# soedinglab/spacedust

Measured on AMD Instinct MI355X. Metric: clustersearch throughput (genome-pairs/s; SW GCUPS alongside), higher is better.
Workload: dtype int16

## Files before the change

include/spacedust_gpu.h:

```cpp
#ifndef SPACEDUST_GPU_H
#define SPACEDUST_GPU_H

#include <stddef.h>
#include <stdint.h>

#ifdef __cplusplus
extern "C" {
#endif

enum {
    SD_OK = 0,
    SD_ENODEVICE = -1,
    SD_EHIP = -2,
    SD_EINVAL = -3,
    SD_ENOMEM = -4,
    SD_EUNSUPPORTED = -5,
    SD_EMISMATCH = -6
};

typedef struct sd_ctx sd_ctx;
typedef struct sd_seqset sd_seqset;
typedef struct sd_target sd_target;

int sd_ctx_create(int device, sd_ctx **out);
// ... 48 lines not shown
                              uint32_t nPairs, const uint32_t *pairQ, const uint32_t *pairT, const uint8_t *isIdentity,
                              uint32_t *outIdx, sd_sw_result *out, uint32_t *nOut, char *btPool, uint64_t btCap,
                              uint64_t *btUsed);

int sd_sw_align_batch_compact_diag(sd_ctx *ctx, const sd_sw_params *par, const sd_seqset *queries, const sd_seqset *targets,
                                   uint32_t nPairs, const uint32_t *pairQ, const uint32_t *pairT, const uint16_t *pairDiag,
                                   const uint8_t *isIdentity, uint32_t *outIdx, sd_sw_result *out, uint32_t *nOut, char *btPool,
                                   uint64_t btCap, uint64_t *btUsed);

int sd_seqset_set_groups(sd_seqset *s, const uint32_t *groupOf, uint32_t nGroups, const uint32_t *keys);
int sd_sw_align_batch_best_by_group(sd_ctx *ctx, const sd_sw_params *par, const sd_seqset *queries, const sd_seqset *targets,
                                    uint32_t nPairs, const uint32_t *pairQ, const uint32_t *pairT, const uint16_t *pairDiag,
                                    const uint8_t *isIdentity, float seqIdThr, int32_t alnLenThr, uint32_t *outIdx, sd_sw_result *out,
                                    uint32_t *nOut, char *btPool, uint64_t btCap, uint64_t *btUsed);

int sd_sw_align_alt_batch(sd_ctx *ctx, const sd_sw_params *par, const sd_seqset *queries, const sd_seqset *targets, uint32_t nSeeds,
                          const uint32_t *seedQ, const uint32_t *seedT, const int32_t *tStart, const int32_t *tEnd,
                          const uint8_t *isIdentity, uint32_t maxAlt, float seqIdThr, int32_t alnLenThr, int32_t seqIdMode,
                          sd_sw_result *out, uint32_t *outCount, char *btPool, uint64_t btCap, uint64_t *btUsed);
int sd_sw_alt_last_stats(sd_ctx *ctx, uint64_t *groups, uint64_t *seedRounds, uint64_t *bytesCopied);

int sd_sw_set_cigar_pool(sd_ctx *ctx, int on);
int sd_sw_download_bytes(sd_ctx *ctx, uint64_t *recordBytes, uint64_t *poolBytes);

int sd_selftest_sort_pairs(sd_ctx *ctx, const uint32_t *keys, const uint32_t *vals, uint32_t n, int beginBit, int endBit, uint32_t *outKeys,
                           uint32_t *outVals);
int sd_selftest_scan(sd_ctx *ctx, const uint32_t *in, uint32_t n, uint64_t *exclusiveSum, uint32_t *runningMax);
int sd_selftest_r2p_weights(sd_ctx *ctx, uint32_t nTasks, const uint32_t *nRows, const uint32_t *L, const uint8_t *cells, float *freq,
                            float *eff);

int sd_sw_align_batch_hostpath(sd_ctx *ctx, const sd_sw_params *par, const sd_seqset *queries, const sd_seqset *targets,
                               uint32_t nPairs, const uint32_t *pairQ, const uint32_t *pairT, const uint8_t *isIdentity,
                               sd_sw_result *out, char *btPool, uint64_t btCap, uint64_t *btUsed);

int sd_sw_score_batch(sd_ctx *ctx, const sd_sw_params *par, const sd_seqset *queries, const sd_seqset *targets,
                      uint32_t nPairs, const uint32_t *pairQ, const uint32_t *pairT, int lanes, int reverse,
                      const int32_t *qEnd, const int32_t *tEnd, int32_t *out);

int sd_sw_last_cells(sd_ctx *ctx, uint64_t *forwardCells, uint64_t *reverseCells, uint64_t *tracebackCells);

typedef struct {
    int32_t kmerSize;
    int32_t kmerThr;
    int32_t maxHitsPerQuery;
    int32_t minDiagScore;
    uint32_t binSize;
// ... 343 lines not shown
```

spacedust_amd/_lib.py:

```python
import ctypes as C
import os

import numpy as np

HERE = os.path.dirname(os.path.abspath(__file__))
LIB_PATH = os.path.join(HERE, 'libsdgpu.so')

_vp = C.c_void_p


SD_OK, SD_ENODEVICE, SD_EHIP, SD_EINVAL, SD_ENOMEM, SD_EUNSUPPORTED, SD_EMISMATCH = 0, -1, -2, -3, -4, -5, -6


class SdError(RuntimeError):
    pass


class SwParams(C.Structure):
    _fields_ = [('gapOpen', C.c_int32), ('gapExtend', C.c_int32), ('matrix', C.c_int8 * 441), ('covMode', C.c_int32),
                ('covThr', C.c_float), ('evalThr', C.c_double), ('swMode', C.c_int32), ('dbResidues', C.c_uint64)]


class SwResult(C.Structure):
    _fields_ = [('score', C.c_int32), ('qStart', C.c_int32), ('qEnd', C.c_int32), ('tStart', C.c_int32),
# ... 196 lines not shown
        'sd_search_create_indexed': (C.c_int, [C.c_int, C.POINTER(SearchParams), C.POINTER(SetDbView), C.POINTER(IndexView), C.POINTER(_vp)]),
        'sd_search_destroy': (None, [_vp]),
        'sd_search_last_error': (C.c_char_p, [_vp]),
        'sd_search_ctx': (_vp, [_vp, C.c_int]),
        'sd_search_target': (_vp, [_vp]),
        'sd_search_set_sinks': (C.c_int, [_vp, _vp, _vp, _vp]),
        'sd_search_set_chunk_queries': (C.c_int, [_vp, C.c_int32]),
        'sd_search_set_want_records': (C.c_int, [_vp, C.c_int]),
        'sd_search_stream': (C.c_int, [_vp, C.POINTER(SetDbView), C.c_int, C.c_uint32, _vp, _vp, _vp]),
        'sd_search_result_counts': (C.c_int, [_vp, _vp]),
        'sd_search_result_arrays': (C.c_int, [_vp] + [_vp] * 12),
        'sd_search_result_write_tsv': (C.c_int, [_vp, C.c_char_p, C.c_char_p, _vp, C.c_char_p, _vp, C.c_char_p, _vp, C.c_char_p, _vp,
                                                 C.c_int, C.c_int, C.c_uint64, C.POINTER(C.c_uint64), C.POINTER(C.c_uint64)]),
        'sd_search_result_records': (C.c_int, [_vp, _vp, C.c_uint64, C.POINTER(C.c_uint64)]),
        'sd_agg_records': (C.c_int, [_vp] * 7 + [_vp, C.c_uint64, C.POINTER(C.c_uint64)]),
        'sd_records_check': (C.c_int, [_vp, C.c_uint64, C.c_uint32, C.c_uint32, C.c_uint32, C.c_uint32, C.POINTER(C.c_uint64), C.POINTER(C.c_uint64)]),
        'sd_records_write_tsv': (C.c_int, [_vp, C.c_uint64, C.c_char_p, C.c_int, C.c_uint64, C.c_char_p, _vp, C.c_char_p, _vp, C.c_char_p, _vp,
                                           C.c_char_p, _vp, C.c_int, C.POINTER(C.c_uint64), C.POINTER(C.c_uint64)]),
        'sd_search_result_destroy': (None, [_vp]),
        'sd_search_stats': (C.c_int, [_vp, _vp, _vp]),
        'sd_search_download_bytes': (C.c_int, [_vp, C.POINTER(C.c_uint64), C.POINTER(C.c_uint64)]),
        'sd_sw_set_cigar_pool': (C.c_int, [_vp, C.c_int]),
        'sd_sw_download_bytes': (C.c_int, [_vp, C.POINTER(C.c_uint64), C.POINTER(C.c_uint64)]),
        'sd_r2p_create': (C.c_int, [C.POINTER(_vp)]),
        'sd_r2p_destroy': (None, [_vp]),
        'sd_r2p_batch': (C.c_int, [_vp, C.POINTER(R2pParams), C.c_uint32] + [_vp] * 12),
        'sd_r2p_batch_device': (C.c_int, [_vp, _vp, C.POINTER(R2pParams), C.c_uint32] + [_vp] * 12),
        'sd_selftest_r2p_weights': (C.c_int, [_vp, C.c_uint32, _vp, _vp, _vp, _vp, _vp]),
        'sd_shard_query_sets': (C.c_int, [_vp, C.c_uint32, C.c_uint32, C.c_uint32, _vp, C.POINTER(C.c_uint32)]),
        'sd_comm_unique_id': (C.c_int, [C.c_char_p]),
        'sd_comm_init': (C.c_int, [C.c_int, C.c_int, C.c_int, C.c_char_p, C.POINTER(_vp)]),
        'sd_comm_destroy': (None, [_vp]),
        'sd_comm_host_buffer': (C.c_int, [_vp, C.c_int, C.c_uint64, C.POINTER(_vp)]),
        'sd_comm_last_error': (C.c_char_p, [_vp]),
        'sd_search_set_records_sink': (C.c_int, [_vp, _vp, _vp]),
        'sd_gather_stream_begin': (C.c_int, [_vp, C.c_int, C.c_uint32, _vp, C.c_uint32, _vp, C.c_uint64, C.c_int, C.POINTER(_vp)]),
        'sd_gather_stream_end': (C.c_int, [_vp, _vp, _vp, C.POINTER(C.c_uint64)]),
        'sd_gather_stream_begin_tcp': (C.c_int, [_vp, C.c_int, C.c_int, C.c_uint32, _vp, C.c_uint32, _vp, C.c_uint64, C.c_int, C.POINTER(_vp)]),
        'sd_gather_results': (C.c_int, [_vp, _vp, C.c_uint64, C.c_int, _vp, _vp, C.c_uint64, C.POINTER(C.c_uint64)]),
        'sd_tcp_connect': (C.c_int, [C.c_char_p, C.c_int, C.c_int, C.c_int, C.POINTER(_vp)]),
        'sd_tcp_close': (None, [_vp]),
        'sd_tcp_bcast': (C.c_int, [_vp, _vp, C.c_uint64]),
        'sd_tcp_gather': (C.c_int, [_vp, _vp, C.c_uint64, _vp, _vp, C.c_uint64, C.POINTER(C.c_uint64)]),
    }
    missing = []
    for name, (res, args) in sig.items():
# ... 29 lines not shown
```

spacedust_amd/api.py:

```python
import ctypes as C

import numpy as np

from . import _lib
from .cpus import effective_cpus
from ._lib import SdError, ptr


def _check(ctx, rc, what):
    if rc != 0:
        msg = ''
        if ctx is not None:
            msg = _lib.load().sd_last_error(ctx).decode(errors='replace')
        raise SdError('%s failed (%d): %s' % (what, rc, msg))


class Host:

    def __init__(self, threads=0):
        import os
        self.L = _lib.load()
        self.threads = threads or effective_cpus()
        h = C.c_void_p()
        _check(None, self.L.sd_host_create(self.threads, C.byref(h)), 'sd_host_create')
# ... 393 lines not shown
        s = SeqSet(self, res, off, None)
        s.set_letters(blob)
        return s

    def rescore_diagonal(self, host, queries, targets, hit_q, hit_t, hit_diag, mode=2):
        m, _, a2n = host.matrix(0)
        par = _lib.RescoreParams()
        par.mode = int(mode)
        C.memmove(par.matrix, m.ctypes.data, 441)
        C.memmove(par.aa2num, a2n.ctypes.data, 256)
        hq = np.ascontiguousarray(hit_q, np.uint32)
        ht = np.ascontiguousarray(hit_t, np.uint32)
        hd = np.ascontiguousarray(np.asarray(hit_diag, np.int64) & 0xFFFF, np.uint16)
        assert len(hq) == len(ht) == len(hd)
        out = np.zeros(len(hq), _lib.RESCORE_DTYPE)
        _check(self.h, self.L.sd_rescore_diagonal_batch(self.h, C.byref(par), queries.h, targets.h, len(hq), ptr(hq), ptr(ht), ptr(hd),
                                                        ptr(out)), 'sd_rescore_diagonal_batch')
        return out

    def set_cigar_pool(self, on=True):
        _check(self.h, self.L.sd_sw_set_cigar_pool(self.h, 1 if on else 0), 'sd_sw_set_cigar_pool')
        self._cigar_pool = bool(on)

    def sw_download_bytes(self):
        a, b = C.c_uint64(), C.c_uint64()
        self.L.sd_sw_download_bytes(self.h, C.byref(a), C.byref(b))
        return a.value, b.value

    def sw_cells(self):
        f, r, t = C.c_uint64(), C.c_uint64(), C.c_uint64()
        self.L.sd_sw_last_cells(self.h, C.byref(f), C.byref(r), C.byref(t))
        return f.value, r.value, t.value

    def __del__(self):
        try:
            h, self.h = self.h, None
            if h:
                self.L.sd_ctx_destroy(h)
        except Exception:
            pass


class SeqSet:
    def __init__(self, ctx, residues, offsets, sw_bias, aln=None):
        self.ctx = ctx
        self.residues = np.ascontiguousarray(residues, np.uint8)
# ... 225 lines not shown
```

spacedust_amd/csrc/cli/sd_mod_iter.cpp:

```cpp
#include "sd_align_core.h"
#include "sd_cli.h"
#include "sd_pref_core.h"

#include <algorithm>
#include <atomic>
#include <chrono>
#include <climits>
#include <cmath>
#include <condition_variable>
#include <cstdio>
#include <cstdlib>
#include <cstring>
#include <memory>
#include <mutex>
#include <omp.h>
#include <string>
#include <sys/resource.h>
#include <thread>
#include <vector>

namespace sdcli {

namespace {

// ... 33 lines not shown
    bool sameDb = false;
    int numIt = 1, device = 0;
    sd_target *seqTarget = nullptr, *profTarget = nullptr;
    sd_seqset *tset = nullptr;
    PrefSetup pfSeq, pfProf;
    AlignSetup alFirst, alMid, alLast;
    const R2pSetup *r2p = nullptr;
    double subtractEval = 0.001;
    bool profile = false;
};

struct Worker {
    sd_ctx *ctx = nullptr;
    sd_host *host = nullptr;
    sd_r2p *r2p = nullptr;
    int threads = 1;
    QueryChunk Q;
    std::vector<uint8_t> failed;
    AlignChunk C;
    std::vector<uint32_t> mark;
    uint32_t stamp = 0;
    ~Worker() {
        if (r2p) sd_r2p_destroy(r2p);
        if (ctx) sd_ctx_destroy(ctx);
        if (host) sd_host_destroy(host);
    }
};

double quantE(double v) {
    char text[32];
    double back = v;
    sd_host_quantise_3e(v, text, &back);
    return back;
}

int failChunk(ChunkOut &o, int rc, const std::string &what, sd_ctx *ctx) {
    o.rc = rc;
    o.err = what + " failed (" + std::to_string(rc) + ")";
    if (ctx) o.err += std::string(": ") + sd_last_error(ctx);
    return rc;
}

int processChunk(const Shared &S, Worker &W, uint32_t g0, uint32_t g1, ChunkOut &out) {
    const SeqDb &qdb = *S.qdb, &tdb = *S.tdb;
    const uint32_t nq = g1 - g0;
    out.g0 = g0;
// ... 237 lines not shown
    if (int rc = alignSetupFromArgs(alnArgs(eUser, false), host.h, tdb->totalResidues(), S.alLast)) return rc;
    R2pSetup RS;
    if (int rc = r2pSetupFromArgs(subArgs("result2profile", profFlags, &err), RS)) return rc;
    S.r2p = &RS;
    {
        const double eU = strtod(eUser.c_str(), nullptr), eP = strtod(eProfile.c_str(), nullptr);
        S.subtractEval = eU < eP ? eU : eP;
    }

    int nWorkers = getenv("SD_ITER_WORKERS") ? atoi(getenv("SD_ITER_WORKERS")) : 4;
    nWorkers = std::max(1, std::min(nWorkers, 8));
    uint32_t chunkQ = (uint32_t) std::max<long long>(1, a.integer("--iter-chunk-queries", getenv("SD_ITER_CHUNK") ? atoi(getenv("SD_ITER_CHUNK")) : 1500));
    const int perWorker = std::max(1, std::min(threads, (threads * 3 / 2 + nWorkers - 1) / nWorkers));
    std::vector<std::unique_ptr<Worker> > workers;
    for (int w = 0; w < nWorkers; w++) {
        workers.emplace_back(new Worker());
        Worker &W = *workers.back();
        W.threads = perWorker;
        int rc = sd_ctx_create(device, &W.ctx);
        if (rc != SD_OK) return failNoDevice(rc);
        if (sd_host_create(perWorker, &W.host) != SD_OK) return fail("sd_host_create failed");
        if (sd_r2p_create(&W.r2p) != SD_OK) return fail("sd_r2p_create failed");
        if (S.profile) sd_profile_enable(W.ctx, 1);
    }
    uint64_t indexEntries = 0;
    TargetH seqTarget, profTarget;
    SeqSetH tset;
    {
        sd_ctx *c0 = workers[0]->ctx;
        uint64_t st[2] = {0, 0};
        if (int rc = buildTarget(host.h, c0, S.pfSeq, tdb->residues.data(), tdb->offsets.data(), tdb->n, &seqTarget.t, st)) return rc;
        indexEntries = st[0];
        info(a, "Index table k-mer threshold: %d at k-mer size %d\nIndex statistics\nEntries:          %llu\n", S.pfSeq.kmerThr, S.pfSeq.k,
             (unsigned long long) st[0]);
        if (numIt > 1) {
            if (int rc = buildTarget(host.h, c0, S.pfProf, tdb->residues.data(), tdb->offsets.data(), tdb->n, &profTarget.t, st, std::string(),
                                     "sd_target_build (profile searches)"))
                return rc;
            indexEntries = std::max<uint64_t>(indexEntries, st[0]);
            info(a, "Index table k-mer threshold: %d at k-mer size %d (profile iterations: every k-mer indexed)\nEntries:          %llu\n",
                 S.pfProf.kmerThr, S.pfProf.k, (unsigned long long) st[0]);
        }
        const int rc = sd_seqset_create(c0, tdb->residues.data(), tdb->offsets.data(), tdb->n, nullptr, &tset.s);
        if (rc != SD_OK) return failCtx(c0, rc, "sd_seqset_create(targets)");
    }
    S.seqTarget = seqTarget.t;
// ... 412 lines not shown
```

spacedust_amd/csrc/hip/sd_common.h:

```cpp
#ifndef SD_COMMON_H
#define SD_COMMON_H

#include <hip/hip_runtime.h>

#include <cstdarg>
#include <cstdint>
#include <cstdio>
#include <cstring>
#include <algorithm>
#include <ctime>
#include <sys/prctl.h>
#include <map>
#include <mutex>
#include <string>
#include <vector>

#include "spacedust_gpu.h"

struct sd_profile_entry {
    double ms = 0.0;
    uint64_t launches = 0;
};

struct sd_ctx {
    int device = 0;
    hipStream_t stream = nullptr;
    std::string lastError;
    bool profiling = false;
    std::map<std::string, sd_profile_entry> profile;
    hipEvent_t evStart = nullptr, evStop = nullptr;
    bool biasTablesUploaded = false;
    hipEvent_t evSync = nullptr;
    uint64_t cellsFwd = 0, cellsRev = 0, cellsTb = 0;
    uint64_t cellsUngapped = 0;
    uint64_t altGroups = 0, altSeedRounds = 0, altBytes = 0;
    const sd_sw_result *alignDevRes = nullptr;
    size_t alignDevResN = 0;
    bool cigarPool = false;
    uint64_t d2hRecordBytes = 0, d2hPoolBytes = 0;
    hipDeviceProp_t prop;
    struct WsEntry { void *p = nullptr; size_t bytes = 0; };
    std::map<std::string, WsEntry> ws;
    std::map<std::string, WsEntry> pinned;
    struct ProfPending { std::string name; hipEvent_t a = nullptr, b = nullptr; };
    std::vector<ProfPending> profPending;
    std::vector<hipEvent_t> evPool;
    struct PoolBuf { void *p = nullptr; size_t bytes = 0; };
    std::vector<PoolBuf> pool;
    std::mutex poolMutex;
    struct BounceBlock { uint8_t *p = nullptr; size_t cap = 0; };
    struct BounceItem { void *dst = nullptr; const uint8_t *src = nullptr; size_t bytes = 0; };
    std::vector<BounceBlock> bounce;
    std::vector<BounceItem> bounceItems;
    size_t bounceCur = 0, bounceUsed = 0;
};

inline hipError_t poolGet(sd_ctx *ctx, size_t bytes, void **out, size_t *got) {
    {
        std::lock_guard<std::mutex> lock(ctx->poolMutex);
        int best = -1;
        for (size_t i = 0; i < ctx->pool.size(); i++)
// ... 306 lines not shown
```

spacedust_amd/csrc/hip/sd_sw.hip:

```cpp
#include "sd_common.h"
#include <unistd.h>


#include <algorithm>
#include <cmath>
#include <cstring>
#include <memory>
#include <omp.h>
#include <numeric>

#include "../host/sd_host.h"
#include "sd_sw_pk.h"

namespace {

using sdpk::SwTask;

template <int RT>
__global__ void __launch_bounds__(64)
sw_score_kernel(const SwTask *__restrict__ tasks, uint32_t nTasks, const uint8_t *__restrict__ qRes,
                const int8_t *__restrict__ qBias, const uint8_t *__restrict__ tRes, const int8_t *__restrict__ mat,
                int go, int ge, int32_t *__restrict__ out, uint2 *__restrict__ boundary,
                const uint32_t *__restrict__ order ,
                const int8_t *__restrict__ qProf ) {
    constexpr int ROWS = 32 * RT;
    constexpr int WORDS = RT / 4;
    __shared__ uint32_t prof[2][21][ROWS / 4];
    __shared__ int8_t smat[441];
    for (int i = threadIdx.x; i < 441; i += 64) smat[i] = mat[i];
    __syncthreads();

    const int grp = threadIdx.x >> 5;
    const int l = threadIdx.x & 31;
    const uint32_t taskId = blockIdx.x * 2 + grp;
    SwTask tk;
    if (taskId < nTasks) {
        tk = tasks[order ? order[taskId] : taskId];
    } else {
        tk.n = 0; tk.tL = 0; tk.qOff = 0; tk.tOff = 0; tk.qStep = 1; tk.tStep = 1; tk.segLen = 1; tk.slot = 0; tk.boundOff = 0;
// ... 854 lines not shown
    double p2 = n_lj_y * P_n_F - sqrt_vj_y * E_n_F;
    double c_y = fmax(e.cThr, e.sigma * y_ + e.tau);
    double area = p1 * p2 + c_y * (P_m_F * P_n_F);
    return e.K * exp(-e.lambda * y_) * area;
}

__device__ __forceinline__ float devCov(unsigned int startPos, unsigned int endPos, unsigned int len) {
    return (min(len, max(startPos, endPos)) - min(startPos, endPos) + 1) / (float) len;
}
__device__ __forceinline__ bool devHasCoverage(float covThr, int covMode, float qCov, float tCov) {
    switch (covMode) {
        case 0: return (qCov >= covThr) && (tCov >= covThr);
        case 2: return qCov >= covThr;
        case 1: return tCov >= covThr;
        default: return true;
    }
}

__global__ void __launch_bounds__(256)
k_pre_word(uint32_t nPairs, const uint32_t *__restrict__ pairQ, const uint32_t *__restrict__ pairT, const uint16_t *__restrict__ pairDiag,
           const uint32_t *__restrict__ fwdKeys, const uint64_t *__restrict__ qOff, const uint64_t *__restrict__ tOff,
           const uint8_t *__restrict__ qRes, const int8_t *__restrict__ qBias, const uint8_t *__restrict__ tRes, const int8_t *__restrict__ mat,
           const int8_t *__restrict__ qProf, const int32_t *__restrict__ minBias, int matMin, uint8_t *__restrict__ preWord,
           uint32_t *__restrict__ pass1Keys) {
    __shared__ int8_t smat[441];
    for (int x = threadIdx.x; x < 441; x += blockDim.x) smat[x] = mat[x];
    __syncthreads();
    const uint32_t i = blockIdx.x * blockDim.x + threadIdx.x;
    if (i >= nPairs) return;
    uint8_t pw = 0;
    const uint32_t key = fwdKeys[i];
    if (key != KEY_INVALID) {
        const uint64_t qo = qOff[pairQ[i]], to = tOff[pairT[i]];
        const int qL = (int) (qOff[pairQ[i] + 1] - qo), tL = (int) (tOff[pairT[i] + 1] - to);
        if (qL < 32768 && tL < 32768 && pairDiag[i] != 0x8000) {
            const int d = (int) (int16_t) pairDiag[i];
            int q0 = d >= 0 ? d : 0, t0 = d >= 0 ? 0 : -d;
            const int n = min(qL - q0, tL - t0);
            const int need = 255 - (abs(matMin) + abs(minBias[pairQ[i]]));
            int run = 0, best = 0;
            for (int x = 0; x < n && best < need; x++) {
                const int qr = qRes[qo + q0 + x], tr = tRes[to + t0 + x];
                run += qProf ? (int) qProf[(qo + q0 + x) * 21 + tr] : (int) smat[tr * 21 + qr] + (int) qBias[qo + q0 + x];
                run = run < 0 ? 0 : run;
                best = run > best ? run : best;
            }
            pw = best >= need ? 1 : 0;
        }
    }
    preWord[i] = pw;
    pass1Keys[i] = pw ? KEY_INVALID : key;
}

__global__ void __launch_bounds__(256)
k_make_fwd(uint32_t nPairs, const uint32_t *__restrict__ pairQ, const uint32_t *__restrict__ pairT,
           const uint8_t *__restrict__ ident, const uint64_t *__restrict__ qOff, const uint64_t *__restrict__ tOff,
           SwTask *__restrict__ tasks, uint32_t *__restrict__ keys, uint32_t *__restrict__ vals,
           sd_sw_result *__restrict__ res, int usePk) {
    const uint32_t i = blockIdx.x * blockDim.x + threadIdx.x;
    if (i >= nPairs) return;
    const uint64_t qo = qOff[pairQ[i]], to = tOff[pairT[i]];
    const int qL = (int) (qOff[pairQ[i] + 1] - qo), tL = (int) (tOff[pairT[i] + 1] - to);
// ... 8 lines not shown
    sd_sw_result r;
    r.score = 0; r.qStart = -1; r.qEnd = -1; r.tStart = -1; r.tEnd = -1; r.identical = 0; r.btLen = 0; r.flags = 0;
    r.evalue = 0.0; r.btOffset = 0;
    res[i] = r;
}

__global__ void k_bounds(const uint32_t *__restrict__ keys, uint32_t n, uint32_t step, uint32_t *__restrict__ b, int nb) {
    const int c = threadIdx.x;
    if (c >= nb) return;
    const uint64_t want = (uint64_t) c * step;
    uint32_t lo = 0, hi = n;
    while (lo < hi) {
        uint32_t mid = (lo + hi) >> 1;
        if ((uint64_t) keys[mid] < want) lo = mid + 1;
        else hi = mid;
    }
    b[c] = lo;
}

__global__ void __launch_bounds__(256)
k_gate_word(uint32_t nPairs, const uint32_t *__restrict__ pairQ, const int32_t *__restrict__ out32,
            const int32_t *__restrict__ minBias, int matMin, SwTask *__restrict__ tasks, uint32_t *__restrict__ keys,
            uint32_t *__restrict__ vals, uint8_t *__restrict__ word, const uint32_t *__restrict__ fwdKeys, int usePk, int wideRowLimit,
            const uint8_t *__restrict__ preWord ) {
    const uint32_t i = blockIdx.x * blockDim.x + threadIdx.x;
    if (i >= nPairs) return;
    vals[i] = i;
    bool w = false;
    if (fwdKeys[i] != KEY_INVALID) {
        const int mb = minBias[pairQ[i]];
        const int bias = abs(matMin) + abs(mb);
        w = (preWord && preWord[i]) || out32[3 * i] + bias >= 255;
    }
    word[i] = w ? 1 : 0;
    if (w) {
        tasks[i].segLen = max(1, (tasks[i].n + 15) / 16);
        keys[i] = scoreKey(tasks[i].n, tasks[i].tL, usePk ? SCORE_PK_WIDE : SCORE_INT32, wideRowLimit);
    } else {
        keys[i] = KEY_INVALID;
    }
}

__global__ void __launch_bounds__(256)
k_gate_rev(uint32_t nPairs, DevGateParams gp, const uint32_t *__restrict__ pairQ, const uint32_t *__restrict__ pairT,
           const uint64_t *__restrict__ qOff, const uint64_t *__restrict__ tOff, const int32_t *__restrict__ out32,
           const int32_t *__restrict__ out16, const uint8_t *__restrict__ word, const uint32_t *__restrict__ fwdKeys,
           SwTask *__restrict__ tasks, uint32_t *__restrict__ keys, uint32_t *__restrict__ vals,
           sd_sw_result *__restrict__ res, int usePk) {
    const uint32_t i = blockIdx.x * blockDim.x + threadIdx.x;
    if (i >= nPairs) return;
    vals[i] = i;
    keys[i] = KEY_INVALID;
    if (fwdKeys[i] == KEY_INVALID) return;
    const int32_t *src = word[i] ? &out16[3 * i] : &out32[3 * i];
    sd_sw_result r = res[i];
    r.score = src[0];
    r.tEnd = src[1];
    r.qEnd = src[2];
    r.flags = word[i] ? 1 : 0;
    if (word[i] && r.tEnd == -1) r.tEnd = 0;
    if (r.score == 0) r.qEnd = 0;
    if (r.tEnd == -1) { res[i] = r; return; }
    const uint64_t qo = qOff[pairQ[i]], to = tOff[pairT[i]];
    const int qL = (int) (qOff[pairQ[i] + 1] - qo), tL = (int) (tOff[pairT[i] + 1] - to);
    const double ev = devEvalue(gp, (double) r.score, (double) qL);
    r.evalue = ev;
    const bool lowE = ev > gp.evalThr * (1.0 + 1e-9);
    const float qCov = devCov(0, r.qEnd, qL), tCov = devCov(0, r.tEnd, tL);
    const bool lowCov = !devHasCoverage(gp.covThr, gp.covMode, qCov, tCov);
    res[i] = r;
    if (gp.swMode == 0 || lowE || lowCov) return;
    SwTask tk;
    tk.qOff = qo + r.qEnd; tk.tOff = to + r.tEnd;
    tk.n = r.qEnd + 1; tk.tL = r.tEnd + 1; tk.qStep = -1; tk.tStep = -1;
    const int lanes = word[i] ? 16 : 32;
    tk.segLen = max(1, (tk.n + lanes - 1) / lanes);
    tk.slot = i; tk.boundOff = 0;
    tasks[i] = tk;
    keys[i] = scoreKey(tk.n, tk.tL, !usePk ? SCORE_INT32 : (word[i] ? SCORE_PK_WIDE : SCORE_PK), gp.wideRowLimit);
}

constexpr int N_TB_NARROW = 9;
__constant__ int c_tbNarrowQ[N_TB_NARROW] = {128, 192, 256, 320, 384, 512, 640, 768, 1024};
static const int TB_NARROW_Q[N_TB_NARROW] = {128, 192, 256, 320, 384, 512, 640, 768, 1024};
__device__ __forceinline__ bool tbNarrow(int band, int qLen, int tLen) { return band * 2 + 3 <= 32 && qLen <= 1024 && tLen <= 1024 + 13; }
__device__ __forceinline__ uint32_t tbKey(int band, int qLen, int tLen) {
    const int w = band * 2 + 3;
    int ci;
    if (tbNarrow(band, qLen, tLen)) {
        ci = 0;
        while (qLen > c_tbNarrowQ[ci]) ci++;
    } else {
        ci = N_TB_NARROW + (w <= 127 ? 0 : (w <= 511 ? 1 : (w <= 2047 ? 2 : 3)));
    }
    if (ci < N_TB_NARROW) {
        const int tries = band <= 1 ? 4 : (band <= 3 ? 3 : (band <= 7 ? 2 : 1));
        return (uint32_t) ci * 4096u + (uint32_t) (4 - tries) * 1024u + (uint32_t) (1023 - min(max(qLen - 1, 0), 1023));
    }
    const unsigned long long work = (unsigned long long) ((2 * band + 1 + 31) / 32) * (unsigned long long) qLen;
    return (uint32_t) ci * 4096u + (uint32_t) (4095 - (int) min(work >> 3, 4095ull));
}
constexpr uint32_t N_TB_CLASSES = N_TB_NARROW + 4;
// ... 937 lines not shown
    SD_HIP(ctx, wsGet(ctx, "al.btlen", N + 1, &dBtLen));
    SD_HIP(ctx, wsGet(ctx, "al.dense", N + 1, &dDense));
    SD_HIP(ctx, wsGet(ctx, "al.cells", 4, &dCells));
    SD_HIP(ctx, hipMemcpyAsync(dMat, par->matrix, 441, hipMemcpyHostToDevice, ctx->stream));
    SD_HIP(ctx, hipMemcpyAsync(dPQ, pairQ, N * sizeof(uint32_t), hipMemcpyHostToDevice, ctx->stream));
    SD_HIP(ctx, hipMemcpyAsync(dPT, pairT, N * sizeof(uint32_t), hipMemcpyHostToDevice, ctx->stream));
    if (isIdentity) SD_HIP(ctx, hipMemcpyAsync(dIdent, isIdentity, N, hipMemcpyHostToDevice, ctx->stream));
    else SD_HIP(ctx, hipMemsetAsync(dIdent, 0, N, ctx->stream));
    SD_HIP(ctx, hipMemcpyAsync(dMinBias, queries->dProf ? queries->hProfBias.data() : queries->hMinBias.data(),
                               queries->n * sizeof(int32_t), hipMemcpyHostToDevice, ctx->stream));
    SD_HIP(ctx, hipMemsetAsync(dErr, 0, 4 * sizeof(int), ctx->stream));
    SD_HIP(ctx, hipMemsetAsync(dCells, 0, 4 * sizeof(unsigned long long), ctx->stream));
    SD_HIP(ctx, hipMemsetAsync(dOut32, 0, N * 3 * sizeof(int32_t), ctx->stream));
    SD_HIP(ctx, hipMemsetAsync(dOut16, 0, N * 3 * sizeof(int32_t), ctx->stream));
    SD_HIP(ctx, hipMemsetAsync(dOutRev, 0, N * 3 * sizeof(int32_t), ctx->stream));
    SD_HIP(ctx, hipMemsetAsync(dBtLen, 0, (N + 1) * sizeof(uint64_t), ctx->stream));

    hs.reset(new HostScope(ctx, "align.fwd32"));
    const int usePk = (go >= ge && go < 1024 && ge >= 0 && getenv("SD_SW_INT32") == nullptr) ? 1 : 0;
    uint32_t nValid = 0;
    hipLaunchKernelGGL(k_make_fwd, dim3(grid), dim3(256), 0, ctx->stream, nPairs, dPQ, dPT, dIdent, queries->dOff, targets->dOff,
                       dTasks, dFwdKeys, dVals, dRes, usePk);
    uint32_t *dPass1Keys = dFwdKeys;
    uint8_t *dPreWord = nullptr;
    if (pairDiag && usePk) {
        uint16_t *dDiag = nullptr;
        SD_HIP(ctx, wsGet(ctx, "al.diag", N, &dDiag));
        SD_HIP(ctx, wsGet(ctx, "al.preword", N, &dPreWord));
        SD_HIP(ctx, wsGet(ctx, "al.pass1keys", N, &dPass1Keys));
        SD_HIP(ctx, hipMemcpyAsync(dDiag, pairDiag, N * sizeof(uint16_t), hipMemcpyHostToDevice, ctx->stream));
        hipLaunchKernelGGL(k_pre_word, dim3(grid), dim3(256), 0, ctx->stream, nPairs, (const uint32_t *) dPQ, (const uint32_t *) dPT,
                           (const uint16_t *) dDiag, (const uint32_t *) dFwdKeys, (const uint64_t *) queries->dOff, (const uint64_t *) targets->dOff,
                           (const uint8_t *) queries->dRes, (const int8_t *) queries->dBias, (const uint8_t *) targets->dRes, (const int8_t *) dMat,
                           (const int8_t *) queries->dProf, (const int32_t *) dMinBias, queries->dProf ? 0 : matMin, dPreWord, dPass1Keys);
    }
    hipLaunchKernelGGL(k_cells, dim3(grid), dim3(256), 0, ctx->stream, nPairs, dTasks, dPass1Keys, dCells + 0);
    const uint32_t *dShare = queries->n >= (1u << PAIR_QUERY_BITS) ? nullptr : dPQ;
    int rc = devRunScore(ctx, nPairs, dPass1Keys, dVals, dKeysS, dOrder, dBounds, dTasks, dScanA, dScanB, queries, targets, dMat, go,
                         ge, dOut32, &nValid, dShare);
    if (rc != SD_OK) return rc;
    hs.reset(new HostScope(ctx, "align.fwd16"));
    hipLaunchKernelGGL(k_gate_word, dim3(grid), dim3(256), 0, ctx->stream, nPairs, dPQ, dOut32, dMinBias, queries->dProf ? 0 : matMin, dTasks, dKeys,
                       dVals, dWord, dFwdKeys, usePk, gp.wideRowLimit, (const uint8_t *) dPreWord);
    hipLaunchKernelGGL(k_cells, dim3(grid), dim3(256), 0, ctx->stream, nPairs, dTasks, dKeys, dCells + 0);
    rc = devRunScore(ctx, nPairs, dKeys, dVals, dKeysS, dOrder, dBounds, dTasks, dScanA, dScanB, queries, targets, dMat, go, ge,
                     dOut16, &nValid, dShare);
    if (rc != SD_OK) return rc;
    hs.reset(new HostScope(ctx, "align.rev"));
    hipLaunchKernelGGL(k_gate_rev, dim3(grid), dim3(256), 0, ctx->stream, nPairs, gp, dPQ, dPT, queries->dOff, targets->dOff, dOut32,
                       dOut16, dWord, dFwdKeys, dTasks, dRevKeys, dVals, dRes, usePk);
    hipLaunchKernelGGL(k_cells, dim3(grid), dim3(256), 0, ctx->stream, nPairs, dTasks, dRevKeys, dCells + 1);
    rc = devRunScore(ctx, nPairs, dRevKeys, dVals, dKeysS, dOrder, dBounds, dTasks, dScanA, dScanB, queries, targets, dMat, go, ge,
                     dOutRev, &nValid, nullptr);
    if (rc != SD_OK) return rc;
    hs.reset(new HostScope(ctx, "align.traceback"));
    hipLaunchKernelGGL(k_gate_tb, dim3(grid), dim3(256), 0, ctx->stream, nPairs, gp, dPQ, dPT, queries->dOff, targets->dOff, dOutRev,
                       dRevKeys, dTb, dKeys, dVals, dDirBytes, dBtBytes, dRes, dErr);
    SD_HIP(ctx, hipMemsetAsync(dBtBytes + N, 0, sizeof(uint64_t), ctx->stream));
    rc = devExclusiveScan(ctx, dBtBytes, dBtOff, N + 1);
    if (rc != SD_OK) return rc;
    uint64_t btScratch = 0;
    SD_HIP(ctx, sdD2H(ctx, &btScratch, dBtOff + N, sizeof(uint64_t)));
    SD_HIP(ctx, sdStreamSync(ctx));
    char *dBt = nullptr;
    SD_HIP(ctx, wsGet(ctx, "tb.bt", btScratch + 64, &dBt));
    uint64_t SCRATCH_BUDGET = 16ull << 30;
    {
        size_t freeB = 0, totalB = 0;
        if (hipMemGetInfo(&freeB, &totalB) == hipSuccess && totalB > 0)
            SCRATCH_BUDGET = std::max<uint64_t>(1ull << 30, std::min<uint64_t>(totalB / 4, freeB / 3));
        if (const char *e = getenv("SD_TB_BUDGET")) SCRATCH_BUDGET = std::max<uint64_t>(1u << 20, strtoull(e, nullptr, 10));
    }
    uint32_t *dKeysRound = nullptr;
// ... 160 lines not shown
    }
    hs.reset(new HostScope(ctx, "align.download"));
    const bool cigarPool = ctx->cigarPool && btPool != nullptr;
    uint64_t *dCigLen = nullptr;
    if (cigarPool) {
        SD_HIP(ctx, wsGet(ctx, "al.ciglen", N + 1, &dCigLen));
        SD_HIP(ctx, hipMemsetAsync(dCigLen + nPairs, 0, (N + 1 - nPairs) * sizeof(uint64_t), ctx->stream));
        hipLaunchKernelGGL(k_bt_cigar<false>, dim3((nPairs + 3) / 4), dim3(256), 0, ctx->stream, nPairs, (const uint64_t *) dBtLen,
                           (const uint64_t *) nullptr, (const TbTask *) dTb, (const char *) dBt, (char *) nullptr, dCigLen, (sd_sw_result *) nullptr);
    }
    rc = devExclusiveScan(ctx, cigarPool ? dCigLen : dBtLen, dDense, N + 1);
    if (rc != SD_OK) return rc;
    uint64_t poolBytes = 0;
    int hErr[4] = {0, 0, 0, 0};
    unsigned long long hCells[4] = {0, 0, 0, 0};
    SD_HIP(ctx, sdD2H(ctx, &poolBytes, dDense + N, sizeof(uint64_t)));
    SD_HIP(ctx, sdD2H(ctx, hErr, dErr, sizeof(hErr)));
    SD_HIP(ctx, sdD2H(ctx, hCells, dCells, sizeof(hCells)));
    SD_HIP(ctx, sdStreamSync(ctx));
    if (hErr[0] == 1) return sdFail(ctx, SD_EMISMATCH, "Score of forward/backward SW differ (fatal in the reference, StripedSmithWaterman.cpp:466-473)");
    if (hErr[0] == 2) return sdFail(ctx, SD_EHIP, "Trace back error");
    ctx->cellsFwd = hCells[0];
    ctx->cellsRev = hCells[1];
    uint64_t identBytes = 0;
    if (isIdentity && btPool)
        for (uint32_t i = 0; i < nPairs; i++)
            if (isIdentity[i]) identBytes += cigarPool ? 8 : targets->hOff[pairT[i] + 1] - targets->hOff[pairT[i]];
    if (poolBytes > 0 && btPool == nullptr) return sdFail(ctx, SD_EINVAL, "swMode 2 needs a backtrace pool");
    if (poolBytes + identBytes > btCap && btPool) return sdFail(ctx, SD_ENOMEM, "backtrace pool too small");
    char *dPool = nullptr;
    SD_HIP(ctx, wsGet(ctx, "al.pool", poolBytes + 64, &dPool));
    if (poolBytes > 0 && cigarPool)
        hipLaunchKernelGGL(k_bt_cigar<true>, dim3((nPairs + 3) / 4), dim3(256), 0, ctx->stream, nPairs, (const uint64_t *) dBtLen,
                           (const uint64_t *) dDense, (const TbTask *) dTb, (const char *) dBt, dPool, (uint64_t *) nullptr, dRes);
    else if (poolBytes > 0)
        hipLaunchKernelGGL(k_bt_pack, dim3((nPairs + 3) / 4), dim3(256), 0, ctx->stream, nPairs, dBtLen, dDense, dTb, dBt, dPool,
                           (uint64_t) 0, dRes);
    uint32_t nRec = nPairs;
    sd_sw_result *dRecSrc = dRes;
    uint32_t *hIdx = nullptr;
    if (compactIdx) {
        uint8_t *dAcc = nullptr;
        uint64_t *dAccPos = nullptr;
        sd_sw_result *dResC = nullptr;
        uint32_t *dIdxC = nullptr;
        SD_HIP(ctx, wsGet(ctx, "al.acc", N + 1, &dAcc));
// ... 83 lines not shown
                r.btOffset = btPos;
                r.flags = nTxt << 8;
                btPos += (uint64_t) nTxt;
            } else if (btPool) {
                memset(btPool + btPos, 'M', L);
                r.btOffset = btPos;
                btPos += L;
            }
        }
    }
    if (btUsed) *btUsed = btPos;
    ctx->d2hRecordBytes += (uint64_t) nRec * (sizeof(sd_sw_result) + (compactIdx ? sizeof(uint32_t) : 0));
    ctx->d2hPoolBytes += poolBytes;
    hs.reset();
    return SD_OK;
}

int sd_sw_set_cigar_pool(sd_ctx *ctx, int on) {
    if (!ctx) return SD_EINVAL;
    ctx->cigarPool = on != 0;
    return SD_OK;
}

int sd_sw_download_bytes(sd_ctx *ctx, uint64_t *recordBytes, uint64_t *poolBytes) {
    if (!ctx) return SD_EINVAL;
    if (recordBytes) *recordBytes = ctx->d2hRecordBytes;
    if (poolBytes) *poolBytes = ctx->d2hPoolBytes;
    return SD_OK;
}

int sd_sw_align_batch(sd_ctx *ctx, const sd_sw_params *par, const sd_seqset *queries, const sd_seqset *targets,
                      uint32_t nPairs, const uint32_t *pairQ, const uint32_t *pairT, const uint8_t *isIdentity,
                      sd_sw_result *out, char *btPool, uint64_t btCap, uint64_t *btUsed) {
    return alignBatchImpl(ctx, par, queries, targets, nPairs, pairQ, pairT, isIdentity, out, btPool, btCap, btUsed, nullptr, nullptr);
}

int sd_sw_align_batch_compact(sd_ctx *ctx, const sd_sw_params *par, const sd_seqset *queries, const sd_seqset *targets,
                              uint32_t nPairs, const uint32_t *pairQ, const uint32_t *pairT, const uint8_t *isIdentity,
                              uint32_t *outIdx, sd_sw_result *out, uint32_t *nOut, char *btPool, uint64_t btCap,
                              uint64_t *btUsed) {
    if (!outIdx || !nOut) return SD_EINVAL;
    return alignBatchImpl(ctx, par, queries, targets, nPairs, pairQ, pairT, isIdentity, out, btPool, btCap, btUsed, outIdx, nOut);
}

int sd_sw_align_batch_compact_diag(sd_ctx *ctx, const sd_sw_params *par, const sd_seqset *queries, const sd_seqset *targets,
                                   uint32_t nPairs, const uint32_t *pairQ, const uint32_t *pairT, const uint16_t *pairDiag,
// ... 323 lines not shown
```

spacedust_amd/csrc/hip/sd_sw_pk.h:

```cpp
#ifndef SD_SW_PK_H
#define SD_SW_PK_H

#include <hip/hip_runtime.h>
#include <cstdint>

namespace sdpk {

struct SwTask {
    uint64_t qOff;
    uint64_t tOff;
    int32_t n;
    int32_t tL;
    int32_t qStep;
    int32_t tStep;
    int32_t segLen;
    uint32_t slot;
    uint64_t boundOff;
};

typedef short s16x2 __attribute__((ext_vector_type(2)));
typedef unsigned short u16x2 __attribute__((ext_vector_type(2)));

__device__ __forceinline__ uint32_t pkMax(uint32_t a, uint32_t b) {
    return __builtin_bit_cast(uint32_t, __builtin_elementwise_max(__builtin_bit_cast(s16x2, a), __builtin_bit_cast(s16x2, b)));
}
__device__ __forceinline__ uint32_t pkSubSat(uint32_t a, uint32_t b) {
    return __builtin_bit_cast(uint32_t, __builtin_elementwise_sub_sat(__builtin_bit_cast(u16x2, a), __builtin_bit_cast(u16x2, b)));
}
__device__ __forceinline__ uint32_t pkSub(uint32_t a, uint32_t b) {
    return __builtin_bit_cast(uint32_t, (s16x2) (__builtin_bit_cast(s16x2, a) - __builtin_bit_cast(s16x2, b)));
}
__device__ __forceinline__ uint32_t pkAdd(uint32_t a, uint32_t b) {
    return __builtin_bit_cast(uint32_t, (s16x2) (__builtin_bit_cast(s16x2, a) + __builtin_bit_cast(s16x2, b)));
}
__device__ __forceinline__ uint32_t pkLshr(uint32_t a, int s) {
    return __builtin_bit_cast(uint32_t, (u16x2) (__builtin_bit_cast(u16x2, a) >> (u16x2) ((unsigned short) s)));
}
__device__ __forceinline__ uint32_t pkAshr(uint32_t a, int s) {
    return __builtin_bit_cast(uint32_t, (s16x2) (__builtin_bit_cast(s16x2, a) >> (s16x2) ((short) s)));
}
__device__ __forceinline__ uint32_t pkRowCode(uint32_t g, int code) {
    uint32_t r;
    asm("v_pk_mad_i16 %0, %1, 32, %2 op_sel_hi:[1,0,0] clamp" : "=v"(r) : "v"(g), "s"(code));
    return r;
}
__device__ __forceinline__ uint32_t bfi(uint32_t mask, uint32_t a, uint32_t b) { return (a & mask) | (b & ~mask); }

__device__ __forceinline__ void addProfile4(uint32_t pa, uint32_t pb, uint32_t d0, uint32_t d1, uint32_t d2, uint32_t d3,
                                            uint32_t &h0, uint32_t &h1, uint32_t &h2, uint32_t &h3) {
    asm("v_add_u16_sdwa %0, %4, sext(%8) dst_sel:WORD_0 dst_unused:UNUSED_PAD src0_sel:WORD_0 src1_sel:BYTE_0\n\t"
        "v_add_u16_sdwa %1, %5, sext(%8) dst_sel:WORD_0 dst_unused:UNUSED_PAD src0_sel:WORD_0 src1_sel:BYTE_1\n\t"
        "v_add_u16_sdwa %2, %6, sext(%8) dst_sel:WORD_0 dst_unused:UNUSED_PAD src0_sel:WORD_0 src1_sel:BYTE_2\n\t"
        "v_add_u16_sdwa %3, %7, sext(%8) dst_sel:WORD_0 dst_unused:UNUSED_PAD src0_sel:WORD_0 src1_sel:BYTE_3\n\t"
        "v_add_u16_sdwa %0, %4, sext(%9) dst_sel:WORD_1 dst_unused:UNUSED_PRESERVE src0_sel:WORD_1 src1_sel:BYTE_0\n\t"
        "v_add_u16_sdwa %1, %5, sext(%9) dst_sel:WORD_1 dst_unused:UNUSED_PRESERVE src0_sel:WORD_1 src1_sel:BYTE_1\n\t"
        "v_add_u16_sdwa %2, %6, sext(%9) dst_sel:WORD_1 dst_unused:UNUSED_PRESERVE src0_sel:WORD_1 src1_sel:BYTE_2\n\t"
        "v_add_u16_sdwa %3, %7, sext(%9) dst_sel:WORD_1 dst_unused:UNUSED_PRESERVE src0_sel:WORD_1 src1_sel:BYTE_3\n\t"
        "s_nop 0"
        : "=&v"(h0), "=&v"(h1), "=&v"(h2), "=&v"(h3)
        : "v"(d0), "v"(d1), "v"(d2), "v"(d3), "v"(pa), "v"(pb));
}

__device__ __forceinline__ uint32_t dppShr1(uint32_t v) {
// ... 522 lines not shown
```

spacedust_amd/csrc/host/sd_search.cpp:

```cpp
#include "sd_host.h"
#include "sd_target_build.h"
#include "spacedust_gpu.h"

#include <algorithm>
#include <chrono>
#include <condition_variable>
#include <cstdio>
#include <cstdlib>
#include <cstring>
#include <deque>
#include <fstream>
#include <functional>
#include <future>
#include <memory>
#include <mutex>
#include <string>
#include <thread>
#include <pthread.h>
#include <vector>

namespace {

double nowSec() {
    return std::chrono::duration<double>(std::chrono::steady_clock::now().time_since_epoch()).count();
// ... 429 lines not shown
    if (profile && (!Q->sortedScore || !Q->sortedIndex)) return SD_EINVAL;
    const double tAll = nowSec();
    const sd_setdb &T = s->T;
    std::vector<int32_t> qLen(Q->n);
    for (uint32_t i = 0; i < Q->n; i++) qLen[i] = (int32_t) (Q->offsets[i + 1] - Q->offsets[i]);
    const bool aggregate = Q->setId && Q->posInSet && Q->strand && T.setId && T.posInSet && T.strand;
    const bool pushdown = aggregate && !s->alnSink && !(getenv("SD_EVAL_PUSHDOWN") && atoi(getenv("SD_EVAL_PUSHDOWN")) == 0);
    s->swParRun = s->swPar;
    if (pushdown) s->swParRun.evalThr = std::min(s->swPar.evalThr, 1.2e-6);
    s->stats[S_EVAL_PUSHDOWN] = pushdown ? 1 : 0;
    s->bestOnDevice = pushdown && s->targetHasGroups && !(getenv("SD_BEST_ON_DEVICE") && atoi(getenv("SD_BEST_ON_DEVICE")) == 0);
    s->cigarOnDevice = aggregate && !s->alnSink && !(getenv("SD_CIGAR_ON_DEVICE") && atoi(getenv("SD_CIGAR_ON_DEVICE")) == 0);
    struct CigarMode {
        sd_ctx *al[4];
        explicit CigarMode(sd_search *s_, bool on) : al{s_->ctxAl, s_->ctxAl2, s_->ctxAlMore[0], s_->ctxAlMore[1]} {
            for (sd_ctx *c : al)
                if (c) sd_sw_set_cigar_pool(c, on ? 1 : 0);
        }
        ~CigarMode() {
            for (sd_ctx *c : al)
                if (c) sd_sw_set_cigar_pool(c, 0);
        }
    } cigarMode(s, s->cigarOnDevice);
    std::vector<uint32_t> qSetSize(Q->nSets, 0);
    if (aggregate)
        for (uint32_t i = 0; i < Q->n; i++)
            if (Q->setId[i] < Q->nSets) qSetSize[Q->setId[i]]++;
    if (aggregate) {
        uint32_t m = 0;
        for (uint32_t v : qSetSize) m = std::max(m, v);
        for (uint32_t v : s->tSetSize) m = std::max(m, v);
        for (uint32_t i = 0; i < Q->n; i++) m = std::max(m, Q->posInSet[i]);
        for (uint32_t i = 0; i < T.n; i++) m = std::max(m, T.posInSet[i]);
        if (s->lgamma.size() < (size_t) m + 8) {
            s->lgamma.resize((size_t) m + 8);
            sd_host_lgamma_table(s->lgamma.data(), (uint32_t) s->lgamma.size());
        }
    }
    std::vector<std::unique_ptr<sd_search_result> > res(nRanges);
    for (uint32_t r = 0; r < nRanges; r++) {
        res[r].reset(new sd_search_result());
        if (!aggregate) continue;
        int rc = sd_agg_create(Q->setId, qLen.data(), Q->n, T.setId, s->tLen.data(), T.n, Q->nSets, T.nSets, s->par.evalThr, s->par.covMode,
                               s->par.covThr, s->par.alnLenThr, s->par.filterSelfMatch, &res[r]->agg);
        if (rc != SD_OK) return s->fail(rc, "sd_agg_create");
        if (Q->keys || T.keys) sd_agg_set_keys(res[r]->agg, Q->keys, T.keys);
// ... 578 lines not shown
```

Baseline: 2858.

## Skip wide forward rerun for word-overflow pairs whose narrow score is exact

Adds a narrow-final mode, on by default, in which pairs that overflow the byte-range gate are only rerun with the wider packed forward scorer when their 32-bit pass score reaches a fixed exactness threshold (1023), come from the prefilter, or have very long targets. Otherwise the reverse pass reuses the first-pass score. The prefilter's ungapped-run threshold is also raised to that constant, so fewer pairs get pre-marked as wide. The aim is to cut the second forward scoring pass for most word pairs. It adds a wave ballot with atomic counters for profiling statistics and depends on the first-pass score being exact below the threshold.

Measured after the change: 2907 (median of 6 runs). 1.02x the previous value.

```diff
diff --git a/include/spacedust_gpu.h b/include/spacedust_gpu.h
--- a/include/spacedust_gpu.h
+++ b/include/spacedust_gpu.h
@@ -94,6 +94,8 @@
 
 int sd_sw_set_cigar_pool(sd_ctx *ctx, int on);
 int sd_sw_download_bytes(sd_ctx *ctx, uint64_t *recordBytes, uint64_t *poolBytes);
+
+int sd_sw_set_narrow_final(sd_ctx *ctx, int on);
 
 int sd_selftest_sort_pairs(sd_ctx *ctx, const uint32_t *keys, const uint32_t *vals, uint32_t n, int beginBit, int endBit, uint32_t *outKeys,
                            uint32_t *outVals);
diff --git a/spacedust_amd/_lib.py b/spacedust_amd/_lib.py
--- a/spacedust_amd/_lib.py
+++ b/spacedust_amd/_lib.py
@@ -242,6 +242,7 @@
         'sd_search_download_bytes': (C.c_int, [_vp, C.POINTER(C.c_uint64), C.POINTER(C.c_uint64)]),
         'sd_sw_set_cigar_pool': (C.c_int, [_vp, C.c_int]),
         'sd_sw_download_bytes': (C.c_int, [_vp, C.POINTER(C.c_uint64), C.POINTER(C.c_uint64)]),
+        'sd_sw_set_narrow_final': (C.c_int, [_vp, C.c_int]),
         'sd_r2p_create': (C.c_int, [C.POINTER(_vp)]),
         'sd_r2p_destroy': (None, [_vp]),
         'sd_r2p_batch': (C.c_int, [_vp, C.POINTER(R2pParams), C.c_uint32] + [_vp] * 12),
diff --git a/spacedust_amd/api.py b/spacedust_amd/api.py
--- a/spacedust_amd/api.py
+++ b/spacedust_amd/api.py
@@ -439,6 +439,9 @@
         _check(self.h, self.L.sd_sw_set_cigar_pool(self.h, 1 if on else 0), 'sd_sw_set_cigar_pool')
         self._cigar_pool = bool(on)
 
+    def set_narrow_final(self, on=True):
+        _check(self.h, self.L.sd_sw_set_narrow_final(self.h, 1 if on else 0), 'sd_sw_set_narrow_final')
+
     def sw_download_bytes(self):
         a, b = C.c_uint64(), C.c_uint64()
         self.L.sd_sw_download_bytes(self.h, C.byref(a), C.byref(b))
diff --git a/spacedust_amd/csrc/cli/sd_mod_iter.cpp b/spacedust_amd/csrc/cli/sd_mod_iter.cpp
--- a/spacedust_amd/csrc/cli/sd_mod_iter.cpp
+++ b/spacedust_amd/csrc/cli/sd_mod_iter.cpp
@@ -79,6 +79,7 @@
     uint32_t stamp = 0;
     ~Worker() {
         if (r2p) sd_r2p_destroy(r2p);
+        if (ctx) sd_sw_set_narrow_final(ctx, 0);
         if (ctx) sd_ctx_destroy(ctx);
         if (host) sd_host_destroy(host);
     }
@@ -362,6 +363,7 @@
         if (sd_host_create(perWorker, &W.host) != SD_OK) return fail("sd_host_create failed");
         if (sd_r2p_create(&W.r2p) != SD_OK) return fail("sd_r2p_create failed");
         if (S.profile) sd_profile_enable(W.ctx, 1);
+        sd_sw_set_narrow_final(W.ctx, (getenv("SD_SW_NARROW_FINAL") && atoi(getenv("SD_SW_NARROW_FINAL")) == 0) ? 0 : 1);
     }
     uint64_t indexEntries = 0;
     TargetH seqTarget, profTarget;
diff --git a/spacedust_amd/csrc/hip/sd_common.h b/spacedust_amd/csrc/hip/sd_common.h
--- a/spacedust_amd/csrc/hip/sd_common.h
+++ b/spacedust_amd/csrc/hip/sd_common.h
@@ -37,6 +37,7 @@
     const sd_sw_result *alignDevRes = nullptr;
     size_t alignDevResN = 0;
     bool cigarPool = false;
+    bool narrowFinal = false;
     uint64_t d2hRecordBytes = 0, d2hPoolBytes = 0;
     hipDeviceProp_t prop;
     struct WsEntry { void *p = nullptr; size_t bytes = 0; };
diff --git a/spacedust_amd/csrc/hip/sd_sw.hip b/spacedust_amd/csrc/hip/sd_sw.hip
--- a/spacedust_amd/csrc/hip/sd_sw.hip
+++ b/spacedust_amd/csrc/hip/sd_sw.hip
@@ -15,6 +15,7 @@
 namespace {
 
 using sdpk::SwTask;
+using sdpk::NARROW_EXACT;
 
 template <int RT>
 __global__ void __launch_bounds__(64)
@@ -915,7 +916,7 @@
            const uint32_t *__restrict__ fwdKeys, const uint64_t *__restrict__ qOff, const uint64_t *__restrict__ tOff,
            const uint8_t *__restrict__ qRes, const int8_t *__restrict__ qBias, const uint8_t *__restrict__ tRes, const int8_t *__restrict__ mat,
            const int8_t *__restrict__ qProf, const int32_t *__restrict__ minBias, int matMin, uint8_t *__restrict__ preWord,
-           uint32_t *__restrict__ pass1Keys) {
+           uint32_t *__restrict__ pass1Keys, int narrowFinal) {
     __shared__ int8_t smat[441];
     for (int x = threadIdx.x; x < 441; x += blockDim.x) smat[x] = mat[x];
     __syncthreads();
@@ -930,7 +931,7 @@
             const int d = (int) (int16_t) pairDiag[i];
             int q0 = d >= 0 ? d : 0, t0 = d >= 0 ? 0 : -d;
             const int n = min(qL - q0, tL - t0);
-            const int need = 255 - (abs(matMin) + abs(minBias[pairQ[i]]));
+            const int need = narrowFinal ? NARROW_EXACT : 255 - (abs(matMin) + abs(minBias[pairQ[i]]));
             int run = 0, best = 0;
             for (int x = 0; x < n && best < need; x++) {
                 const int qr = qRes[qo + q0 + x], tr = tRes[to + t0 + x];
@@ -985,22 +986,31 @@
 k_gate_word(uint32_t nPairs, const uint32_t *__restrict__ pairQ, const int32_t *__restrict__ out32,
             const int32_t *__restrict__ minBias, int matMin, SwTask *__restrict__ tasks, uint32_t *__restrict__ keys,
             uint32_t *__restrict__ vals, uint8_t *__restrict__ word, const uint32_t *__restrict__ fwdKeys, int usePk, int wideRowLimit,
-            const uint8_t *__restrict__ preWord ) {
+            const uint8_t *__restrict__ preWord ,
+            uint8_t *__restrict__ wide ,
+            unsigned long long *__restrict__ wordCount ) {
     const uint32_t i = blockIdx.x * blockDim.x + threadIdx.x;
-    if (i >= nPairs) return;
-    vals[i] = i;
-    bool w = false;
-    if (fwdKeys[i] != KEY_INVALID) {
-        const int mb = minBias[pairQ[i]];
-        const int bias = abs(matMin) + abs(mb);
-        w = (preWord && preWord[i]) || out32[3 * i] + bias >= 255;
-    }
-    word[i] = w ? 1 : 0;
-    if (w) {
-        tasks[i].segLen = max(1, (tasks[i].n + 15) / 16);
-        keys[i] = scoreKey(tasks[i].n, tasks[i].tL, usePk ? SCORE_PK_WIDE : SCORE_INT32, wideRowLimit);
-    } else {
-        keys[i] = KEY_INVALID;
+    bool w = false, rerun = false;
+    if (i < nPairs) {
+        vals[i] = i;
+        if (fwdKeys[i] != KEY_INVALID) {
+            const int mb = minBias[pairQ[i]];
+            const int bias = abs(matMin) + abs(mb);
+            const bool pre = preWord && preWord[i];
+            w = pre || out32[3 * i] + bias >= 255;
+            rerun = w && (!wide || pre || out32[3 * i] >= NARROW_EXACT || tasks[i].tL > 65535);
+        }
+        word[i] = w ? 1 : 0;
+        if (wide) wide[i] = rerun ? 1 : 0;
+        if (w) tasks[i].segLen = max(1, (tasks[i].n + 15) / 16);
+        keys[i] = rerun ? scoreKey(tasks[i].n, tasks[i].tL, usePk ? SCORE_PK_WIDE : SCORE_INT32, wideRowLimit) : KEY_INVALID;
+    }
+    if (wide) {
+        const int nw = __popcll(__ballot(w)), nr = __popcll(__ballot(rerun));
+        if ((threadIdx.x & (warpSize - 1)) == 0 && nw) {
+            atomicAdd(&wordCount[0], (unsigned long long) nw);
+            if (nr) atomicAdd(&wordCount[1], (unsigned long long) nr);
+        }
     }
 }
 
@@ -1009,13 +1019,15 @@
            const uint64_t *__restrict__ qOff, const uint64_t *__restrict__ tOff, const int32_t *__restrict__ out32,
            const int32_t *__restrict__ out16, const uint8_t *__restrict__ word, const uint32_t *__restrict__ fwdKeys,
            SwTask *__restrict__ tasks, uint32_t *__restrict__ keys, uint32_t *__restrict__ vals,
-           sd_sw_result *__restrict__ res, int usePk) {
+           sd_sw_result *__restrict__ res, int usePk,
+           const uint8_t *__restrict__ wide ) {
     const uint32_t i = blockIdx.x * blockDim.x + threadIdx.x;
     if (i >= nPairs) return;
     vals[i] = i;
     keys[i] = KEY_INVALID;
     if (fwdKeys[i] == KEY_INVALID) return;
-    const int32_t *src = word[i] ? &out16[3 * i] : &out32[3 * i];
+    const bool rerun = wide ? wide[i] != 0 : word[i] != 0;
+    const int32_t *src = rerun ? &out16[3 * i] : &out32[3 * i];
     sd_sw_result r = res[i];
     r.score = src[0];
     r.tEnd = src[1];
@@ -1040,7 +1052,7 @@
     tk.segLen = max(1, (tk.n + lanes - 1) / lanes);
     tk.slot = i; tk.boundOff = 0;
     tasks[i] = tk;
-    keys[i] = scoreKey(tk.n, tk.tL, !usePk ? SCORE_INT32 : (word[i] ? SCORE_PK_WIDE : SCORE_PK), gp.wideRowLimit);
+    keys[i] = scoreKey(tk.n, tk.tL, !usePk ? SCORE_INT32 : (rerun ? SCORE_PK_WIDE : SCORE_PK), gp.wideRowLimit);
 }
 
 constexpr int N_TB_NARROW = 9;
@@ -2024,7 +2036,9 @@
     hipLaunchKernelGGL(k_make_fwd, dim3(grid), dim3(256), 0, ctx->stream, nPairs, dPQ, dPT, dIdent, queries->dOff, targets->dOff,
                        dTasks, dFwdKeys, dVals, dRes, usePk);
     uint32_t *dPass1Keys = dFwdKeys;
-    uint8_t *dPreWord = nullptr;
+    uint8_t *dPreWord = nullptr, *dWide = nullptr;
+    const bool narrowFinal = ctx->narrowFinal && usePk;
+    if (narrowFinal) SD_HIP(ctx, wsGet(ctx, "al.wide", N, &dWide));
     if (pairDiag && usePk) {
         uint16_t *dDiag = nullptr;
         SD_HIP(ctx, wsGet(ctx, "al.diag", N, &dDiag));
@@ -2034,7 +2048,8 @@
         hipLaunchKernelGGL(k_pre_word, dim3(grid), dim3(256), 0, ctx->stream, nPairs, (const uint32_t *) dPQ, (const uint32_t *) dPT,
                            (const uint16_t *) dDiag, (const uint32_t *) dFwdKeys, (const uint64_t *) queries->dOff, (const uint64_t *) targets->dOff,
                            (const uint8_t *) queries->dRes, (const int8_t *) queries->dBias, (const uint8_t *) targets->dRes, (const int8_t *) dMat,
-                           (const int8_t *) queries->dProf, (const int32_t *) dMinBias, queries->dProf ? 0 : matMin, dPreWord, dPass1Keys);
+                           (const int8_t *) queries->dProf, (const int32_t *) dMinBias, queries->dProf ? 0 : matMin, dPreWord, dPass1Keys,
+                           narrowFinal ? 1 : 0);
     }
     hipLaunchKernelGGL(k_cells, dim3(grid), dim3(256), 0, ctx->stream, nPairs, dTasks, dPass1Keys, dCells + 0);
     const uint32_t *dShare = queries->n >= (1u << PAIR_QUERY_BITS) ? nullptr : dPQ;
@@ -2043,14 +2058,14 @@
     if (rc != SD_OK) return rc;
     hs.reset(new HostScope(ctx, "align.fwd16"));
     hipLaunchKernelGGL(k_gate_word, dim3(grid), dim3(256), 0, ctx->stream, nPairs, dPQ, dOut32, dMinBias, queries->dProf ? 0 : matMin, dTasks, dKeys,
-                       dVals, dWord, dFwdKeys, usePk, gp.wideRowLimit, (const uint8_t *) dPreWord);
+                       dVals, dWord, dFwdKeys, usePk, gp.wideRowLimit, (const uint8_t *) dPreWord, dWide, dCells + 2);
     hipLaunchKernelGGL(k_cells, dim3(grid), dim3(256), 0, ctx->stream, nPairs, dTasks, dKeys, dCells + 0);
     rc = devRunScore(ctx, nPairs, dKeys, dVals, dKeysS, dOrder, dBounds, dTasks, dScanA, dScanB, queries, targets, dMat, go, ge,
                      dOut16, &nValid, dShare);
     if (rc != SD_OK) return rc;
     hs.reset(new HostScope(ctx, "align.rev"));
     hipLaunchKernelGGL(k_gate_rev, dim3(grid), dim3(256), 0, ctx->stream, nPairs, gp, dPQ, dPT, queries->dOff, targets->dOff, dOut32,
-                       dOut16, dWord, dFwdKeys, dTasks, dRevKeys, dVals, dRes, usePk);
+                       dOut16, dWord, dFwdKeys, dTasks, dRevKeys, dVals, dRes, usePk, (const uint8_t *) dWide);
     hipLaunchKernelGGL(k_cells, dim3(grid), dim3(256), 0, ctx->stream, nPairs, dTasks, dRevKeys, dCells + 1);
     rc = devRunScore(ctx, nPairs, dRevKeys, dVals, dKeysS, dOrder, dBounds, dTasks, dScanA, dScanB, queries, targets, dMat, go, ge,
                      dOutRev, &nValid, nullptr);
@@ -2257,6 +2272,15 @@
     if (hErr[0] == 2) return sdFail(ctx, SD_EHIP, "Trace back error");
     ctx->cellsFwd = hCells[0];
     ctx->cellsRev = hCells[1];
+    if (narrowFinal && ctx->profiling) {
+        const double add[3] = {(double) hCells[2], (double) hCells[3], (double) (hCells[2] - hCells[3])};
+        static const char *const names[3] = {"stat.sw_word_pairs", "stat.sw_word_wide", "stat.sw_word_narrow_final"};
+        for (int x = 0; x < 3; x++) {
+            sd_profile_entry &pe = ctx->profile[names[x]];
+            pe.ms += add[x];
+            pe.launches += 1;
+        }
+    }
     uint64_t identBytes = 0;
     if (isIdentity && btPool)
         for (uint32_t i = 0; i < nPairs; i++)
@@ -2386,6 +2410,12 @@
     return SD_OK;
 }
 
+int sd_sw_set_narrow_final(sd_ctx *ctx, int on) {
+    if (!ctx) return SD_EINVAL;
+    ctx->narrowFinal = on != 0;
+    return SD_OK;
+}
+
 int sd_sw_download_bytes(sd_ctx *ctx, uint64_t *recordBytes, uint64_t *poolBytes) {
     if (!ctx) return SD_EINVAL;
     if (recordBytes) *recordBytes = ctx->d2hRecordBytes;
diff --git a/spacedust_amd/csrc/hip/sd_sw_pk.h b/spacedust_amd/csrc/hip/sd_sw_pk.h
--- a/spacedust_amd/csrc/hip/sd_sw_pk.h
+++ b/spacedust_amd/csrc/hip/sd_sw_pk.h
@@ -39,6 +39,7 @@
 __device__ __forceinline__ uint32_t pkAshr(uint32_t a, int s) {
     return __builtin_bit_cast(uint32_t, (s16x2) (__builtin_bit_cast(s16x2, a) >> (s16x2) ((short) s)));
 }
+constexpr int NARROW_EXACT = 1023;
 __device__ __forceinline__ uint32_t pkRowCode(uint32_t g, int code) {
     uint32_t r;
     asm("v_pk_mad_i16 %0, %1, 32, %2 op_sel_hi:[1,0,0] clamp" : "=v"(r) : "v"(g), "s"(code));
diff --git a/spacedust_amd/csrc/host/sd_search.cpp b/spacedust_amd/csrc/host/sd_search.cpp
--- a/spacedust_amd/csrc/host/sd_search.cpp
+++ b/spacedust_amd/csrc/host/sd_search.cpp
@@ -475,6 +475,17 @@
                 if (c) sd_sw_set_cigar_pool(c, 0);
         }
     } cigarMode(s, s->cigarOnDevice);
+    struct NarrowFinalMode {
+        sd_ctx *al[4];
+        explicit NarrowFinalMode(sd_search *s_, bool on) : al{s_->ctxAl, s_->ctxAl2, s_->ctxAlMore[0], s_->ctxAlMore[1]} {
+            for (sd_ctx *c : al)
+                if (c) sd_sw_set_narrow_final(c, on ? 1 : 0);
+        }
+        ~NarrowFinalMode() {
+            for (sd_ctx *c : al)
+                if (c) sd_sw_set_narrow_final(c, 0);
+        }
+    } narrowFinalMode(s, !(getenv("SD_SW_NARROW_FINAL") && atoi(getenv("SD_SW_NARROW_FINAL")) == 0));
     std::vector<uint32_t> qSetSize(Q->nSets, 0);
     if (aggregate)
         for (uint32_t i = 0; i < Q->n; i++)
```
